# intcomp/camouflaged-vlm

Hardware: AMD Instinct MI355X
Metric: images/sec at 1024x1024 (SAM-ViT-H + CLIP ViT-L/14), full cascade (higher is better)
Workload: dtype f16 hi.hi MFMA + block-scaled e4m3 MFMA for the two correction products (3 mantissa bits) in the ViT-H qkv / lin1 / lin2 and CLIP MLP GEMMs; 3x f16 split MFMA in the other GEMMs; f32 accumulate; ViT-H attention: q.k^T = ONE f16 product (Q and K as single f16 values), P.v = 2x f16 (P a single f16, V

## Files before the change

camouflaged-vlm_amd/csrc/attention_win2.hip:

```cpp
#include <stdlib.h>
#include <type_traits>
#include "common.h"
#include "../../include/cvlm.h"

namespace {

constexpr float LOG2E = 1.4426950408889634f;
typedef float f32x2 __attribute__((ext_vector_type(2)));

template <int OFF>
__device__ __forceinline__ half4 lds_read_tr16(unsigned lds_addr) {
    half4 r;
    asm volatile("ds_read_b64_tr_b16 %0, %1 offset:%2" : "=v"(r) : "v"(lds_addr), "n"(OFF));
    return r;
}
__device__ __forceinline__ void lds_wait() {
    asm volatile("s_waitcnt lgkmcnt(0)" ::: "memory");
    __builtin_amdgcn_sched_barrier(0);
}
template <int N> __device__ __forceinline__ void wait_vm() { asm volatile("s_waitcnt vmcnt(%0)" ::"n"(N) : "memory"); }
__device__ __forceinline__ void step_barrier() {
    asm volatile("s_waitcnt lgkmcnt(0)" ::: "memory");
    __builtin_amdgcn_s_barrier();
    asm volatile("" ::: "memory");
}

struct OneHotImage2 { half_t v[224 * 32]; };
constexpr OneHotImage2 make_onehot_image2() {
    OneHotImage2 im{};
    for (int s = 0; s < 224; ++s)
        for (int c = 0; c < 32; ++c) {
            const int kh = s / 14, kw = s % 14;
            const bool one = s < 196 && (c == kh || c == 16 + kw);
            const int chunk = (c >> 3) ^ ((s >> 2) & 3);
            im.v[s * 32 + chunk * 8 + (c & 7)] = one ? (half_t)1.0f : (half_t)0.0f;
        }
    return im;
}
__device__ const OneHotImage2 g_onehot2 = make_onehot_image2();

#ifdef CVLM_PROBES
__device__ unsigned long long* g_win2_trace = nullptr;
#define WIN2_STAMP(x) do { if (trace) { __builtin_amdgcn_sched_barrier(0); x = wall_clock64(); __builtin_amdgcn_sched_barrier(0); } } while (0)
#else
#define WIN2_STAMP(x) do { } while (0)
#endif

template <bool PLO, bool QLO, bool KLO>
__global__ __launch_bounds__(512, 1) void attn_win14p_kernel(const cvlm_attn_args g, const int nwx, const int npairs) {
    constexpr int HD = 80, KS = 5, NDB = 5, CPR = 10, KP = 80, VP = 80, L = 14, S_SEQ = 196;
    constexpr int KT = 32, NKT = 7, NCW = 7;
    constexpr int PLANE_B = 5120, SLOT_B = 2 * PLANE_B, IPP = 5;
    constexpr int OFF_K = 0, OFF_V = 3 * SLOT_B, OFF_T = 6 * SLOT_B;
    constexpr int RT_B = 27 * HD * 2, RS_PIECES = (4 * RT_B + 1023) / 1024, RS_B = RS_PIECES * 1024;
    constexpr int OFF_OH = OFF_T + RS_B, OH_B = 224 * 32 * 2;
    constexpr int OFF_TOK = OFF_OH + OH_B, TOK_B = 2 * 224 * 8;
    constexpr int TP = 17, OFF_TAUG = OFF_TOK + 2 * TOK_B;

    extern __shared__ __attribute__((aligned(16))) unsigned char smem[];
    const int tid = threadIdx.x, lane = tid & 63;
    const int wave = __builtin_amdgcn_readfirstlane(tid >> 6);
    const int qc = lane & 31, half = lane >> 5;
    const int D = g.heads * HD;
    const half_t* qkv_hi = (const half_t*)g.qkv_hi;
    const half_t* qkv_lo = (const half_t*)g.qkv_lo;
    const half_t* pad_hi = (const half_t*)g.pad_hi;
    const half_t* pad_lo = (const half_t*)g.pad_lo;
    const int64_t qkv_plane = qkv_lo - qkv_hi, pad_plane = pad_lo - pad_hi;
    const int nwin = nwx * nwx;
    const int SI = g.grid * g.grid;
    const QkvStrides QS = qkv_strides(g.qkv_layout, SI, g.B, g.heads, HD);
    const int my_items = blockIdx.x < npairs ? (npairs - 1 - (int)blockIdx.x) / (int)gridDim.x + 1 : 0;
    const int T = my_items * NKT;
    auto pair_of = [&](int k) -> int { return (int)blockIdx.x + k * (int)gridDim.x; };
    auto token_of = [&](int pair, int slot) -> int {
        const int seq = pair / g.heads;
        const int w = seq % nwin;
        const int wy = w / nwx, wx = w - wy * nwx;
        const int iy = slot / L, ix = slot - iy * L;
        const int y = wy * L + iy, x = wx * L + ix;
        if (y >= g.grid || x >= g.grid) return -1;
        return y * g.grid + x;
    };

    if (wave == NCW) {
        long long* tokoff = (long long*)(smem + OFF_TOK);
        auto fill_tokoff = [&](int k) {
            const int pair = pair_of(k);
            const int head = pair % g.heads, b = (pair / g.heads) / nwin;
            long long* tk = tokoff + (k & 1) * (TOK_B / 8);
            const long long pad_delta = pad_hi - qkv_hi;
#pragma unroll
            for (int r = 0; r < 4; ++r) {
                const int sl = lane + 64 * r;
                if (sl < 224) {
                    const int tok = token_of(pair, sl < S_SEQ ? sl : S_SEQ - 1);
                    const long long ko = tok < 0 ? pad_delta + D + head * HD : (long long)qkv_offset(QS, b, tok, 1, head);
                    tk[sl] = ko | (tok < 0 ? 1 : 0);
                    tk[224 + sl] = (ko + (tok < 0 ? (long long)D : (long long)QS.sop)) | (tok < 0 ? 1 : 0);
                }
            }
            asm volatile("s_waitcnt lgkmcnt(0)" ::: "memory");
        };
        int row_s[IPP], ch_s[IPP];
#pragma unroll
        for (int sub = 0; sub < IPP; ++sub) {
            const int c = sub * 64 + lane;
            row_s[sub] = c / CPR;
            ch_s[sub] = c - row_s[sub] * CPR;
        }
        auto issue_tile = [&](int op, int gt) {
            const int k = gt / NKT, t = gt - k * NKT;
            const long long* tk = tokoff + (k & 1) * (TOK_B / 8) + op * 224 + t * KT;
            unsigned char* dst = smem + (op ? OFF_V : OFF_K) + (gt % 3) * SLOT_B;
            const half_t* src[IPP][2];
#pragma unroll
            for (int sub = 0; sub < IPP; ++sub) {
                const long long ko = tk[row_s[sub]];
                const long long disp = (ko & 1) ? pad_plane : qkv_plane;
                src[sub][0] = qkv_hi + ((ko & ~7ll) + ch_s[sub] * 8);
                src[sub][1] = src[sub][0] + disp;
            }
#pragma unroll
            for (int pl = 0; pl < 2; ++pl) {
                if (!KLO && pl == 1 && op == 0) continue;
#pragma unroll
                for (int sub = 0; sub < IPP; ++sub) glds16(src[sub][pl], dst + pl * PLANE_B + sub * 1024);
            }
        };
        {
            const unsigned char* t0 = (const unsigned char*)g.relh_hi;
            const unsigned char* t1 = (const unsigned char*)g.relh_lo;
            const unsigned char* t2 = (const unsigned char*)g.relw_hi;
            const unsigned char* t3 = (const unsigned char*)g.relw_lo;
#pragma unroll 1
            for (int i = 0; i < RS_PIECES; ++i) {
                int byte = i * 1024 + lane * 16;
                if (byte >= 4 * RT_B) byte = 0;
                const int tbl = byte / RT_B, off = byte - tbl * RT_B;
                const unsigned char* src = (tbl == 0 ? t0 : (tbl == 1 ? t1 : (tbl == 2 ? t2 : t3))) + off;
                glds16(src, smem + OFF_T + i * 1024);
            }
            const unsigned char* oh = (const unsigned char*)g_onehot2.v;
#pragma unroll 1
            for (int i = 0; i < OH_B / 1024; ++i) glds16(oh + i * 1024 + lane * 16, smem + OFF_OH + i * 1024);
        }
        if (T > 0) {
            fill_tokoff(0);
            issue_tile(0, 0);
            if (T > 1) issue_tile(0, 1);
            if (T > 2) issue_tile(0, 2);
            issue_tile(1, 0);
            if (T > 1) issue_tile(1, 1);
        }
        wait_vm<0>();
        step_barrier();
#pragma unroll 1
        for (int gt = 0; gt < T; ++gt) {
            step_barrier();
            const int kn = gt + 3, vn = gt + 2;
            if (kn < T && kn % NKT == 0) fill_tokoff(kn / NKT);
#if defined(CVLM_WIN2_PROBE) && CVLM_WIN2_PROBE == 2
            const bool ik = false, iv = false;
#else
            const bool ik = kn < T, iv = vn < T;
#endif
            if (ik) issue_tile(0, kn);
            if (iv) issue_tile(1, vn);
            constexpr int KB = (KLO ? 2 : 1) * IPP, VB = 2 * IPP;
            if (ik && iv) wait_vm<KB + VB>();
            else if (ik) wait_vm<KB>();
            else if (iv) wait_vm<VB>();
            else wait_vm<0>();
        }
        return;
    }

    float* Taug = (float*)(smem + OFF_TAUG);
    const half_t* OH = (const half_t*)(smem + OFF_OH);
    auto k_slot = [&](int gt) -> const unsigned char* { return smem + OFF_K + (gt % 3) * SLOT_B; };
    auto v_slot = [&](int gt) -> const unsigned char* { return smem + OFF_V + (gt % 3) * SLOT_B; };
    const int tg = lane >> 4, ti = lane & 15;
    const int v_lane_off = (16 * (tg & 1) + 4 * (tg >> 1) + (ti >> 2)) * VP + 4 * (ti & 3);
    typedef std::integral_constant<bool, false> no_c;
    typedef std::integral_constant<bool, true> yes_c;
    bool first = true;
    const int qslot = wave * 32 + qc;
    const bool qvalid = qslot < S_SEQ;
    const int qs = qvalid ? qslot : S_SEQ - 1;
    half8 qn_h[KS], qn_l[KS];
    auto load_q = [&](int pair) {
        const int head = pair % g.heads, b = (pair / g.heads) / nwin;
        const int qtok = token_of(pair, qs);
        const int64_t qo = qtok < 0 ? (int64_t)head * HD : qkv_offset(QS, b, qtok, 0, head);
        const half_t* bh = (qtok < 0 ? pad_hi : qkv_hi) + qo;
        const half_t* bl = bh + (qtok < 0 ? pad_plane : qkv_plane);
#pragma unroll
        for (int ks = 0; ks < KS; ++ks) {
            qn_h[ks] = *(const half8*)(bh + 16 * ks + 8 * half);
            qn_l[ks] = *(const half8*)(bl + 16 * ks + 8 * half);
        }
    };
    if (my_items > 0) load_q(pair_of(0));
#ifdef CVLM_PROBES
    unsigned long long* const trace = g_win2_trace;
    unsigned long long ta = 0, tb = 0, tc = 0, td = 0, acc_u = 0, acc_t = 0, acc_o = 0, acc_bar = 0, t_first = 0;
#endif

#pragma unroll 1
    for (int k = 0; k < my_items; ++k) {
        const int pair = pair_of(k);
        const int head = pair % g.heads, b = (pair / g.heads) / nwin;
        const int gt0 = k * NKT;
        half8 qh[KS + 2], ql[KS + 2];
#pragma unroll
        for (int ks = 0; ks < KS; ++ks) { qh[ks] = qn_h[ks]; ql[ks] = qn_l[ks]; }
        if (first) { step_barrier(); first = false; }
        WIN2_STAMP(ta);
        {
            const int qhh = qs / L, qww = qs - qhh * L;
            float* Tq = Taug + (wave * 32 + qc) * TP;
            if (half == 0) { Tq[14] = 0.f; Tq[15] = 0.f; }
            const int rr = qc < 27 ? qc : 26;
            floatx16 u[2];
#pragma unroll
            for (int tb = 0; tb < 2; ++tb) {
                const unsigned char* rt = smem + OFF_T + (2 * tb) * RT_B + rr * (HD * 2) + 16 * half;
#pragma unroll
                for (int r = 0; r < 16; ++r) u[tb][r] = 0.f;
#pragma unroll
                for (int ks = 0; ks < KS; ++ks) {
                    const half8 rh = *(const half8*)(rt + 32 * ks);
                    const half8 rl = *(const half8*)(rt + RT_B + 32 * ks);
                    u[tb] = __builtin_amdgcn_mfma_f32_32x32x16_f16(rh, qh[ks], u[tb], 0, 0, 0);
                    u[tb] = __builtin_amdgcn_mfma_f32_32x32x16_f16(rl, qh[ks], u[tb], 0, 0, 0);
                    u[tb] = __builtin_amdgcn_mfma_f32_32x32x16_f16(rh, ql[ks], u[tb], 0, 0, 0);
                }
            }
            if (g.scale != 1.0f) {
#pragma unroll
                for (int ks = 0; ks < KS; ++ks)
#pragma unroll
                    for (int j = 0; j < 8; ++j) {
                        half_t hh, ll;
                        split_h2(((float)qh[ks][j] + (float)ql[ks][j]) * g.scale, hh, ll);
                        qh[ks][j] = hh;
                        ql[ks][j] = ll;
                    }
            }
#pragma unroll
            for (int tb = 0; tb < 2; ++tb) {
                int cq = tb ? qww : qhh;
                asm volatile("" : "+v"(cq), "+v"(u[tb][0]));
#pragma unroll
                for (int r = 0; r < 16; ++r) {
                    const int j = (r & 3) + 8 * (r >> 2) + 4 * half;
                    const int kidx = cq + L - 1 - j;
                    const bool ok = j < 27 && kidx >= 0 && kidx < L;
                    Tq[ok ? kidx : 16] = u[tb][r];
                }
                __builtin_amdgcn_wave_barrier();
                {
                    typedef unsigned u32x4_s __attribute__((ext_vector_type(4)));
                    u32x4_s h4, l4;
#pragma unroll
                    for (int j = 0; j < 4; ++j) {
                        unsigned a, b;
                        split_h2_pk(Tq[8 * half + 2 * j], Tq[8 * half + 2 * j + 1], a, b);
                        h4[j] = a; l4[j] = b;
                    }
                    qh[KS + tb] = __builtin_bit_cast(half8, h4);
                    ql[KS + tb] = __builtin_bit_cast(half8, l4);
                }
                __builtin_amdgcn_wave_barrier();
            }
        }

        WIN2_STAMP(tb);
        float m_run = -INFINITY, l_run = 0.f;
        floatx4 o[NDB][2];
#pragma unroll
        for (int n = 0; n < NDB; ++n)
#pragma unroll
            for (int qb = 0; qb < 2; ++qb) o[n][qb] = floatx4{0.f, 0.f, 0.f, 0.f};
        floatx4 osum[2] = {floatx4{0.f, 0.f, 0.f, 0.f}, floatx4{0.f, 0.f, 0.f, 0.f}};

        auto scores = [&](int t, auto last_c) -> floatx16 {
            floatx16 s;
#pragma unroll
            for (int r = 0; r < 16; ++r) s[r] = 0.f;
            const half_t* kr = (const half_t*)k_slot(gt0 + t) + qc * KP + 8 * half;
#pragma unroll
            for (int ks = 0; ks < KS; ++ks) {
                const half8 kh = *(const half8*)(kr + 16 * ks);
                s = __builtin_amdgcn_mfma_f32_32x32x16_f16(kh, qh[ks], s, 0, 0, 0);
                if constexpr (KLO) {
                    const half8 kl = *(const half8*)(kr + PLANE_B / 2 + 16 * ks);
                    s = __builtin_amdgcn_mfma_f32_32x32x16_f16(kl, qh[ks], s, 0, 0, 0);
                }
                if constexpr (QLO) s = __builtin_amdgcn_mfma_f32_32x32x16_f16(kh, ql[ks], s, 0, 0, 0);
            }
            const int row = t * KT + qc;
            const half_t* ohr = OH + row * 32;
#pragma unroll
            for (int a = 0; a < 2; ++a) {
                const half8 oh8 = *(const half8*)(ohr + 8 * ((half + 2 * a) ^ ((row >> 2) & 3)));
                s = __builtin_amdgcn_mfma_f32_32x32x16_f16(oh8, qh[KS + a], s, 0, 0, 0);
                s = __builtin_amdgcn_mfma_f32_32x32x16_f16(oh8, ql[KS + a], s, 0, 0, 0);
            }
            if (decltype(last_c)::value) {
                const int b0 = t * KT + 4 * half;
#pragma unroll
                for (int r = 0; r < 16; ++r)
                    if (b0 + (r & 3) + 8 * (r >> 2) >= S_SEQ) s[r] = -INFINITY;
            }
            return s;
        };
        floatx16 s_cur = scores(0, no_c{});

        auto tile = [&](int t, auto has_next_c, auto next_last_c) {
            constexpr bool HAS_NEXT = decltype(has_next_c)::value;
#ifdef CVLM_PROBES
            unsigned long long te = 0, tf = 0;
            WIN2_STAMP(te);
#endif
            step_barrier();
#ifdef CVLM_PROBES
            WIN2_STAMP(tf);
            if (trace) acc_bar += tf - te;
#endif
#if defined(CVLM_WIN2_PROBE) && CVLM_WIN2_PROBE == 1
            return;
#endif
            floatx16 s_next;
            if (HAS_NEXT) s_next = scores(t + 1, next_last_c);
            const unsigned vaddr = (unsigned)(size_t)(LDS_AS const unsigned char*)v_slot(gt0 + t) + 2u * (unsigned)v_lane_off;
            auto read_v = [&](auto db_c, half4 (&v0)[2], half4 (&v1)[2]) {
                constexpr int DB = decltype(db_c)::value;
                v0[0] = lds_read_tr16<2 * (16 * DB)>(vaddr);                 v1[0] = lds_read_tr16<2 * (16 * DB + 8 * VP)>(vaddr);
                v0[1] = lds_read_tr16<PLANE_B + 2 * (16 * DB)>(vaddr);       v1[1] = lds_read_tr16<PLANE_B + 2 * (16 * DB + 8 * VP)>(vaddr);
            };
            half4 va0[3][2], va1[3][2], vb0[2][2], vb1[2][2];
            read_v(std::integral_constant<int, 0>{}, va0[0], va1[0]);
            read_v(std::integral_constant<int, 1>{}, va0[1], va1[1]);
            read_v(std::integral_constant<int, 2>{}, va0[2], va1[2]);
            const floatx16 s = s_cur;
            float mx = fmaxf(s[0], s[1]);
#pragma unroll
            for (int r = 2; r < 16; r += 2) mx = fmaxf(fmaxf(mx, s[r]), s[r + 1]);
            mx = half_swap_max(mx);
            constexpr float TAU = 5.0f;
            if (__builtin_amdgcn_ballot_w64(mx > m_run + TAU) != 0) {
                const float m_new = fmaxf(m_run, mx);
                const float alpha = __builtin_amdgcn_exp2f((m_run - m_new) * LOG2E);
                l_run *= alpha;
                const auto ax = __builtin_amdgcn_permlane16_swap(__builtin_bit_cast(unsigned, alpha), __builtin_bit_cast(unsigned, alpha), false, false);
                const float a0 = __builtin_bit_cast(float, (unsigned)ax[0]), a1 = __builtin_bit_cast(float, (unsigned)ax[1]);
#pragma unroll
                for (int n = 0; n < NDB; ++n) { o[n][0] *= a0; o[n][1] *= a1; }
                osum[0] *= a0; osum[1] *= a1;
                m_run = m_new;
            }
            const f32x2 c2 = f32x2{-m_run * LOG2E, -m_run * LOG2E}, l2 = f32x2{LOG2E, LOG2E};
            f32x2 z[8], acc = f32x2{0.f, 0.f};
#pragma unroll
            for (int i = 0; i < 8; ++i) {
                const f32x2 a = f32x2{s[2 * i], s[2 * i + 1]} * l2 + c2;
                z[i] = f32x2{__builtin_amdgcn_exp2f(a.x), __builtin_amdgcn_exp2f(a.y)};
                acc += z[i];
            }
            l_run += acc.x + acc.y;
            typedef unsigned u32x4 __attribute__((ext_vector_type(4)));
            u32x4 xh[2], xl[2];
#pragma unroll
            for (int p2 = 0; p2 < 4; ++p2) {
                const f32x2 e0 = z[p2], e1 = z[4 + p2];
                unsigned h0, h1;
                if constexpr (PLO) {
                    h0 = __builtin_bit_cast(unsigned, __builtin_amdgcn_cvt_pkrtz(e0.x, e0.y));
                    h1 = __builtin_bit_cast(unsigned, __builtin_amdgcn_cvt_pkrtz(e1.x, e1.y));
                    const half2v f0 = __builtin_bit_cast(half2v, h0), f1 = __builtin_bit_cast(half2v, h1);
                    const unsigned l0 = __builtin_bit_cast(unsigned, __builtin_amdgcn_cvt_pkrtz(e0.x - (float)f0[0], e0.y - (float)f0[1]));
                    const unsigned l1 = __builtin_bit_cast(unsigned, __builtin_amdgcn_cvt_pkrtz(e1.x - (float)f1[0], e1.y - (float)f1[1]));
                    const auto rl = __builtin_amdgcn_permlane16_swap(l0, l1, false, false);
                    xl[0][p2] = (unsigned)rl[0]; xl[1][p2] = (unsigned)rl[1];
                } else {
                    h0 = __builtin_bit_cast(unsigned, __builtin_convertvector(e0, half2v));
                    h1 = __builtin_bit_cast(unsigned, __builtin_convertvector(e1, half2v));
                }
                const auto rh = __builtin_amdgcn_permlane16_swap(h0, h1, false, false);
                xh[0][p2] = (unsigned)rh[0]; xh[1][p2] = (unsigned)rh[1];
            }
            auto pv = [&](int db, half4 (&v0)[2], half4 (&v1)[2]) {
                const half8 vh = half8{v0[0][0], v0[0][1], v0[0][2], v0[0][3], v1[0][0], v1[0][1], v1[0][2], v1[0][3]};
                const half8 vl = half8{v0[1][0], v0[1][1], v0[1][2], v0[1][3], v1[1][0], v1[1][1], v1[1][2], v1[1][3]};
#pragma unroll
                for (int qb = 0; qb < 2; ++qb) {
                    const half8 bh = __builtin_bit_cast(half8, xh[qb]), bl = __builtin_bit_cast(half8, xl[qb]);
                    if (!PLO && db == 0) {
                        const half_t one = (half_t)1.0f;
                        osum[qb] = __builtin_amdgcn_mfma_f32_16x16x32_f16(half8{one, one, one, one, one, one, one, one}, bh, osum[qb], 0, 0, 0);
                    }
                    o[db][qb] = __builtin_amdgcn_mfma_f32_16x16x32_f16(vh, bh, o[db][qb], 0, 0, 0);
                    o[db][qb] = __builtin_amdgcn_mfma_f32_16x16x32_f16(vl, bh, o[db][qb], 0, 0, 0);
                    if constexpr (PLO) o[db][qb] = __builtin_amdgcn_mfma_f32_16x16x32_f16(vh, bl, o[db][qb], 0, 0, 0);
                }
            };
            lds_wait();
            read_v(std::integral_constant<int, 3>{}, vb0[0], vb1[0]);
            read_v(std::integral_constant<int, 4>{}, vb0[1], vb1[1]);
            pv(0, va0[0], va1[0]);
            pv(1, va0[1], va1[1]);
            pv(2, va0[2], va1[2]);
            lds_wait();
            pv(3, vb0[0], vb1[0]);
            pv(4, vb0[1], vb1[1]);
            if (HAS_NEXT) s_cur = s_next;
        };
#pragma unroll 1
        for (int t = 0; t < NKT - 2; ++t) tile(t, yes_c{}, no_c{});
        tile(NKT - 2, yes_c{}, yes_c{});
        if (k + 1 < my_items) load_q(pair_of(k + 1));
        tile(NKT - 1, no_c{}, no_c{});
        WIN2_STAMP(tc);

        float invq[2];
        if constexpr (PLO) {
            const float l_tot = half_swap_sum(l_run);
            const float inv = 1.0f / l_tot;
            const auto ix = __builtin_amdgcn_permlane16_swap(__builtin_bit_cast(unsigned, inv), __builtin_bit_cast(unsigned, inv), false, false);
            invq[0] = __builtin_bit_cast(float, (unsigned)ix[0]); invq[1] = __builtin_bit_cast(float, (unsigned)ix[1]);
        } else {
            invq[0] = 1.0f / osum[0][0]; invq[1] = 1.0f / osum[1][0];
        }
        const int g4 = lane >> 4;
#pragma unroll
        for (int qb = 0; qb < 2; ++qb) {
            const int qs2 = wave * 32 + 16 * qb + (lane & 15);
            const int tok2 = token_of(pair, qs2 < S_SEQ ? qs2 : S_SEQ - 1);
            const bool ok2 = qs2 < S_SEQ && tok2 >= 0;
            const int64_t orow = ((int64_t)b * SI + (ok2 ? tok2 : 0)) * D + head * HD;
            half_t* oh = (half_t*)g.out_hi + orow;
            half_t* ol = (half_t*)g.out_lo + orow;
            unsigned ph2[NDB][2][2];
#pragma unroll
            for (int n = 0; n < NDB; ++n) {
                split_h2_pk(o[n][qb][0] * invq[qb], o[n][qb][1] * invq[qb], ph2[n][0][0], ph2[n][1][0]);
                split_h2_pk(o[n][qb][2] * invq[qb], o[n][qb][3] * invq[qb], ph2[n][0][1], ph2[n][1][1]);
            }
#pragma unroll
            for (int pl = 0; pl < 2; ++pl) {
                half_t* dst = pl ? ol : oh;
#pragma unroll
                for (int pr = 0; pr < 2; ++pr) {
                    const auto r0 = __builtin_amdgcn_permlane16_swap(ph2[2 * pr][pl][0], ph2[2 * pr + 1][pl][0], false, false);
                    const auto r1 = __builtin_amdgcn_permlane16_swap(ph2[2 * pr][pl][1], ph2[2 * pr + 1][pl][1], false, false);
                    typedef unsigned u32x4 __attribute__((ext_vector_type(4)));
                    const u32x4 v = u32x4{(unsigned)r0[0], (unsigned)r1[0], (unsigned)r0[1], (unsigned)r1[1]};
                    const int d = (g4 & 1) ? 16 * (2 * pr + 1) + 4 * (g4 - 1) : 16 * (2 * pr) + 4 * g4;
                    if (ok2) *(u32x4*)(dst + d) = v;
                }
                typedef unsigned u32x2 __attribute__((ext_vector_type(2)));
                if (ok2) *(u32x2*)(dst + 64 + 4 * g4) = u32x2{ph2[4][pl][0], ph2[4][pl][1]};
            }
        }
#ifdef CVLM_PROBES
        WIN2_STAMP(td);
        if (trace) { acc_u += tb - ta; acc_t += tc - tb; acc_o += td - tc; if (k == 0) t_first = ta; }
#endif
    }
#ifdef CVLM_PROBES
    if (trace && lane == 0) {
        unsigned long long* o = trace + ((size_t)blockIdx.x * 8 + wave) * 8;
        o[0] = acc_u; o[1] = acc_t; o[2] = acc_o; o[3] = (unsigned long long)my_items; o[4] = t_first; o[5] = td; o[6] = acc_bar;
        o[7] = __builtin_amdgcn_s_getreg((31 << 11) | 4);
    }
#endif
    if (first) step_barrier();
}

}

#ifdef CVLM_PROBES
extern "C" int cvlm_debug_set_attn_win2_trace(void* buf) { return (int)hipMemcpyToSymbol(HIP_SYMBOL(g_win2_trace), &buf, sizeof(buf)); }
#endif

template <bool PLO, bool QLO, bool KLO>
static int launch_win14(const cvlm_attn_args& g, hipStream_t s) {
    constexpr int smem = 6 * 10240 + 17 * 1024 + 224 * 32 * 2 + 2 * (2 * 224 * 8) + 224 * 17 * 4;
    const int nwx = (g.grid + 13) / 14;
    const int npairs = g.heads * g.B * nwx * nwx;
    static bool attr[16] = {};
    if (cvlm_first_on_device(attr))
        (void)hipFuncSetAttribute((const void*)attn_win14p_kernel<PLO, QLO, KLO>, hipFuncAttributeMaxDynamicSharedMemorySize, smem);
    static int cus_[16] = {};
    int dev = 0;
    (void)hipGetDevice(&dev);
    int& cus = cus_[dev & 15];
    if (cus == 0 && hipDeviceGetAttribute(&cus, hipDeviceAttributeMultiprocessorCount, dev) != hipSuccess) cus = 256;
    const int wgs = npairs < cus ? npairs : cus;
    hipLaunchKernelGGL((attn_win14p_kernel<PLO, QLO, KLO>), dim3(wgs), dim3(512), smem, s, g, nwx, npairs);
    CVLM_CHECK_LAUNCH();
    return 0;
}

int cvlm_attention_window14_pc(const cvlm_attn_args& g, hipStream_t s) {
    if (g.split_qk == 3 && g.split_pv == 3) return launch_win14<true, true, true>(g, s);
    if (g.split_qk == 2 && g.split_pv == 2) return launch_win14<false, false, true>(g, s);
    if (g.split_qk == 1 && g.split_pv == 2) return launch_win14<false, false, false>(g, s);
    return CVLM_E_UNSUPPORTED;
}
```

camouflaged-vlm_amd/hip.py:

```python
from __future__ import annotations

import ctypes as C
import functools
import os
from typing import Optional, Tuple

import torch

_PKG = os.path.dirname(os.path.abspath(__file__))
LIB_PATH = os.path.join(_PKG, "lib", "libcvlm_hip.so")

ACT_NONE, ACT_GELU, ACT_QUICKGELU, ACT_RELU, ACT_ABS_POST = 0, 1, 2, 3, 4

_SIGNATURES = {
    "cvlm_abi_version": "i:", "cvlm_target_arch": "z:",
    "cvlm_gemm": "i:Gs", "cvlm_gemm_workspace_bytes": "l:", "cvlm_debug_gemm_plan": "i:GiiI",
    "cvlm_layernorm": "i:plpipppfipppiis",
    "cvlm_add_rows": "i:ppifpppiis",
    "cvlm_ln_stats_merge": "i:pliifpps",
    "cvlm_row_stats_split": "i:pfpppliiils",
    "cvlm_row_stats_split_mx": "i:pfplplplpliiils",
    "cvlm_split_f32": "i:pppls",
    "cvlm_patchify": "i:pipiiiiippis",
    "cvlm_im2col3x3": "i:piiiipps",
    "cvlm_reinterpret_transpose": "i:piiifpps",
    "cvlm_attention": "i:As", "cvlm_attention_workspace_bytes": "l:A",
    "cvlm_small_attention": "i:plplplpliiiiis",
    "cvlm_small_attention_h2": "i:plplplplppliiiiis",
    "cvlm_dense_pe": "i:piips",
    "cvlm_mask_head": "i:pppiiips",
    "cvlm_mask_head_edge": "i:pppiiipps",
    "cvlm_mask_head_multi": "i:pppiiiipps",
    "cvlm_bilinear": "i:piiipiiis",
    "cvlm_clip_assemble": "i:ppppiiiips",
    "cvlm_overwrite_rows": "i:piiiiips",
    "cvlm_gather_rows": "i:piiipips",
    "cvlm_gather_rows_h2": "i:ppfiiipips",
    "cvlm_clip_head": "i:ppfiiipppps",
    "cvlm_topk_select": "i:piiipippps",
    "cvlm_text_assemble": "i:ppippipiiiips",
    "cvlm_clip_head_wide_workspace_bytes": "l:ii",
    "cvlm_clip_head_wide": "i:ppfiiipppppls",
    "cvlm_topk_select_wide": "i:piiipippps",
    "cvlm_expand_blocks": "i:piilpppppps",
    "cvlm_normalize_add": "i:ppiips",
    "cvlm_resample_u8": "i:piiiippiiips",
    "cvlm_u8_to_tensor": "i:piiiiiiiippps",
    "cvlm_mask_to_u8": "i:piiiiips",
    "cvlm_mask_joint_hist": "i:ppiiipps",
    "cvlm_mask_pack": "i:pilippps",
    "cvlm_mask_overlap": "i:piilps",
    "cvlm_mask_components_workspace_bytes": "l:iii",
    "cvlm_mask_components": "i:piiiiiiplpppppps",
    "cvlm_debug_mask_components_host": "i:piiiiiipppppp",
    "cvlm_mask_holes_workspace_bytes": "l:iii",
    "cvlm_mask_holes": "i:piiiiiiplppppps",
    "cvlm_debug_mask_holes_host": "i:piiiiiippppp",
    "cvlm_mask_wfm": "i:ppiiipppps",
    "cvlm_prob_quantise": "i:piiippps",
    "cvlm_prob_moments": "i:ppiiipppps",
    "cvlm_prob_wfm": "i:ppiiipppps",
    "cvlm_topk_accumulate": "i:ppiipps",
}
EXPORTS = list(_SIGNATURES)
ABI_VERSION = 12


class GemmArgs(C.Structure):
    _fields_ = [
        ("a_hi", C.c_void_p), ("a_lo", C.c_void_p), ("lda", C.c_int64), ("stride_a", C.c_int64),
        ("w_hi", C.c_void_p), ("w_lo", C.c_void_p), ("ldw", C.c_int64), ("stride_w", C.c_int64),
        ("bias", C.c_void_p),
        ("residual", C.c_void_p), ("ldr", C.c_int64), ("stride_r", C.c_int64),
        ("out_f32", C.c_void_p), ("ldo", C.c_int64), ("stride_o", C.c_int64),
        ("out_hi", C.c_void_p), ("out_lo", C.c_void_p), ("ldoh", C.c_int64), ("stride_oh", C.c_int64),
        ("M", C.c_int32), ("N", C.c_int32), ("K", C.c_int32), ("batch", C.c_int32),
        ("alpha", C.c_float), ("act", C.c_int32), ("split", C.c_int32),
        ("ps_h", C.c_int32), ("ps_w", C.c_int32), ("ps_c2", C.c_int32),
        ("hm_S", C.c_int32), ("hm_H", C.c_int32), ("hm_hd", C.c_int32),
        ("out_scale", C.c_float), ("workspace", C.c_void_p), ("workspace_bytes", C.c_int64),
        ("ln_stats", C.c_void_p), ("ln_colsum", C.c_void_p), ("ln_eps", C.c_float), ("ln_D", C.c_int32),
        ("res_hi", C.c_void_p), ("res_lo", C.c_void_p), ("ldrh", C.c_int64), ("res_scale", C.c_float),
        ("row_stats", C.c_void_p),
        ("conv_h", C.c_int32), ("conv_w", C.c_int32), ("conv_c", C.c_int32),
        ("w_il", C.c_void_p), ("ldw_il", C.c_int64),
        ("a_il", C.c_int32), ("out_il", C.c_int32), ("res_il", C.c_int32),
        ("a_mx", C.c_int32), ("out_mx", C.c_int32), ("res_mx", C.c_int32),
        ("a_mxs", C.c_void_p), ("lda_s", C.c_int64),
        ("w_mx", C.c_void_p), ("ldw_mx", C.c_int64), ("w_mxs", C.c_void_p), ("ldw_s", C.c_int64),
        ("out_mxs", C.c_void_p), ("ldo_s", C.c_int64), ("ldol", C.c_int64), ("ldrl", C.c_int64),
        ("hm_nolo", C.c_int32),
    ]


class GemmLaunchInfo(C.Structure):
    _fields_ = [(n, C.c_int32) for n in ("n0", "N", "nbx", "nby", "grid_x", "grid_y", "block", "lds_bytes", "group_m", "tail_rem",
                                         "tail_split", "total_blocks", "sk_parts", "uses_workspace")] + [("kernel", C.c_char * 128)]


class GemmPlanInfo(C.Structure):
    _fields_ = [("launches", C.c_int32), ("launch", GemmLaunchInfo * 2)]


class AttnArgs(C.Structure):
    _fields_ = [
        ("qkv_hi", C.c_void_p), ("qkv_lo", C.c_void_p), ("pad_hi", C.c_void_p), ("pad_lo", C.c_void_p),
        ("relh_hi", C.c_void_p), ("relh_lo", C.c_void_p), ("relw_hi", C.c_void_p), ("relw_lo", C.c_void_p),
        ("out_hi", C.c_void_p), ("out_lo", C.c_void_p),
        ("B", C.c_int32), ("S", C.c_int32), ("heads", C.c_int32), ("hd", C.c_int32),
        ("mode", C.c_int32), ("grid", C.c_int32), ("window", C.c_int32), ("causal", C.c_int32),
        ("split_qk", C.c_int32), ("split_pv", C.c_int32), ("scale", C.c_float), ("qkv_layout", C.c_int32),
        ("workspace", C.c_void_p), ("workspace_bytes", C.c_int64), ("q_rows", C.c_int32),
    ]


_CTYPES = {"i": C.c_int32, "l": C.c_int64, "f": C.c_float, "p": C.c_void_p, "s": C.c_void_p, "z": C.c_char_p,
           "G": C.POINTER(GemmArgs), "A": C.POINTER(AttnArgs), "I": C.POINTER(GemmPlanInfo)}
ABI = {name: (_CTYPES[sig[0]], [_CTYPES[c] for c in sig[2:]]) for name, sig in _SIGNATURES.items()}
_STREAMED = frozenset(name for name, sig in _SIGNATURES.items() if sig.endswith("s"))

_lib: Optional[C.CDLL] = None


def load() -> C.CDLL:
    global _lib
    if _lib is not None:
        return _lib
    path = os.environ.get("CVLM_PROBE_LIB") or LIB_PATH
    if not os.path.exists(path):
        raise RuntimeError(
            f"{path} is missing: the HIP kernels are the only compute path of this package. "
            "Build them with `python -c 'import __graft_entry__ as g; g.build()'` (hipcc --offload-arch=gfx950).")
    lib = C.CDLL(path)
    for name, (restype, argtypes) in ABI.items():
        fn = getattr(lib, name)
        fn.restype, fn.argtypes = restype, argtypes
    if lib.cvlm_abi_version() != ABI_VERSION:
        raise RuntimeError(f"{path}: ABI {lib.cvlm_abi_version()}, this binding needs {ABI_VERSION}: rebuild the library")
    _lib = lib
    return lib


def _check(rc: int, what: str) -> None:
    if rc != 0:
        raise RuntimeError(f"{what} failed with code {rc}")


def _p(t: Optional[torch.Tensor]) -> Optional[int]:
    return None if t is None else t.data_ptr()


def _planes(x: Optional["H2"]) -> Tuple[Optional[int], Optional[int]]:
    return (None, None) if x is None else (x.hi.data_ptr(), x.lo.data_ptr())


def _stream() -> Optional[int]:
    return torch.cuda.current_stream().cuda_stream or None


def _call(name: str, *args) -> None:
    fn = getattr(load(), name)
    _check(fn(*args, _stream()) if name in _STREAMED else fn(*args), name)


def _on_current_device(t: torch.Tensor) -> None:
    if t.device.type != "cuda" or t.device.index != torch.cuda.current_device():
        raise RuntimeError(f"tensor on {t.device}, current device is cuda:{torch.cuda.current_device()}: call "
                           "torch.cuda.set_device() first (launches use the current device's stream)")


def gemm_workspace_bytes() -> int:
    return load().cvlm_gemm_workspace_bytes()


def new_gemm_workspace(device) -> torch.Tensor:
    return torch.zeros(gemm_workspace_bytes(), dtype=torch.uint8, device=device)


def gemm_workspace_errors(ws: torch.Tensor) -> int:
# ... 607 lines not shown
```

include/cvlm.h:

```cpp
#ifndef CVLM_H
#define CVLM_H
#include <stdint.h>
#ifdef __cplusplus
extern "C" {
#endif

#define CVLM_ABI_VERSION 12
#define CVLM_E_BADARG (-1)
#define CVLM_E_UNSUPPORTED (-2)
#define CVLM_E_WORKSPACE (-3)

enum { CVLM_ACT_NONE = 0, CVLM_ACT_GELU = 1, CVLM_ACT_QUICKGELU = 2, CVLM_ACT_RELU = 3, CVLM_ACT_ABS_POST = 4 };

int cvlm_abi_version(void);
const char* cvlm_target_arch(void);

typedef struct cvlm_gemm_args {
    const void* a_hi; const void* a_lo; int64_t lda; int64_t stride_a;
    const void* w_hi; const void* w_lo; int64_t ldw; int64_t stride_w;
    const float* bias;
    const float* residual; int64_t ldr; int64_t stride_r;
    float* out_f32; int64_t ldo; int64_t stride_o;
    void* out_hi; void* out_lo; int64_t ldoh; int64_t stride_oh;
    int32_t M, N, K, batch;
    float alpha;
    int32_t act;
    int32_t split;
    int32_t ps_h, ps_w, ps_c2;
    int32_t hm_S, hm_H, hm_hd;
    float out_scale;
    void* workspace;
    int64_t workspace_bytes;
    const float* ln_stats; const float* ln_colsum; float ln_eps; int32_t ln_D;
    const void* res_hi; const void* res_lo; int64_t ldrh; float res_scale;
    float* row_stats;
    int32_t conv_h, conv_w, conv_c;
    const void* w_il; int64_t ldw_il;
    int32_t a_il, out_il, res_il;
    int32_t a_mx, out_mx, res_mx;
    const void* a_mxs; int64_t lda_s;
    const void* w_mx; int64_t ldw_mx; const void* w_mxs; int64_t ldw_s;
    void* out_mxs; int64_t ldo_s; int64_t ldol; int64_t ldrl;
    int32_t hm_nolo;
} cvlm_gemm_args;
int cvlm_gemm(const cvlm_gemm_args* args, void* stream);
int64_t cvlm_gemm_workspace_bytes(void);
typedef struct cvlm_gemm_plan_info {
    int32_t launches;
    struct {
        int32_t n0, N;
        int32_t nbx, nby, grid_x, grid_y, block, lds_bytes;
        int32_t group_m, tail_rem, tail_split, total_blocks, sk_parts, uses_workspace;
        char kernel[128];
    } launch[2];
} cvlm_gemm_plan_info;
int cvlm_debug_gemm_plan(const cvlm_gemm_args* args, int have_ws, int cus, cvlm_gemm_plan_info* out);

int cvlm_layernorm(const float* x, int64_t ldx, const float* add, int32_t add_rows, float* sum_out,
                   const float* gamma, const float* beta, float eps, int32_t act,
                   float* out_f32, void* out_hi, void* out_lo, int32_t M, int32_t D, void* stream);

int cvlm_add_rows(const float* a, const float* b, int32_t b_rows, float scale, float* out_f32,
                  void* out_hi, void* out_lo, int32_t M, int32_t D, void* stream);

#define CVLM_LN_FOLD_MAX_RATIO 128
#define CVLM_WS_WORD_LN_REFUSED 513
int cvlm_ln_stats_merge(const float* pieces, int64_t piece_rows, int32_t M, int32_t D, float eps, float* merged, void* gemm_workspace,
                        void* stream);

int cvlm_row_stats_split(const float* x, float scale, void* out_hi, void* out_lo, float* stats, int64_t stats_rows, int32_t M,
                         int32_t D, int32_t copies, int64_t dst_row_stride, void* stream);
int cvlm_row_stats_split_mx(const float* x, float scale, void* out_img, int64_t ld_img, void* out_scales, int64_t ld_s, void* out_lo,
                            int64_t ld_lo, float* stats, int64_t stats_rows, int32_t M, int32_t D, int32_t copies, int64_t dst_row_stride,
                            void* stream);

int cvlm_split_f32(const float* x, void* out_hi, void* out_lo, int64_t n, void* stream);

int cvlm_patchify(const float* src0, int32_t C0, const float* src1, int32_t C1, int32_t B, int32_t H,
                  int32_t W, int32_t p, void* out_hi, void* out_lo, int32_t ldk, void* stream);

int cvlm_im2col3x3(const float* x, int32_t B, int32_t H, int32_t W, int32_t C, void* out_hi, void* out_lo,
                   void* stream);

int cvlm_reinterpret_transpose(const float* x, int32_t B, int32_t T, int32_t D, float scale, void* out_hi, void* out_lo,
                               void* stream);

typedef struct cvlm_attn_args {
    const void* qkv_hi; const void* qkv_lo;
    const void* pad_hi; const void* pad_lo;
    const void* relh_hi; const void* relh_lo;
    const void* relw_hi; const void* relw_lo;
    void* out_hi; void* out_lo;
    int32_t B, S, heads, hd;
    int32_t mode, grid, window, causal;
    int32_t split_qk, split_pv;
    float scale;
    int32_t qkv_layout;
    void* workspace;
    int64_t workspace_bytes;
    int32_t q_rows;
} cvlm_attn_args;
int cvlm_attention(const cvlm_attn_args* args, void* stream);
int64_t cvlm_attention_workspace_bytes(const cvlm_attn_args* args);

int cvlm_small_attention(const float* q, int64_t ldq, const float* k, int64_t ldk, const float* v, int64_t ldv,
                         float* out, int64_t ldo, int32_t B, int32_t nq, int32_t nk, int32_t heads, int32_t hd,
                         void* stream);
int cvlm_small_attention_h2(const float* q, int64_t ldq, const float* k, int64_t ldk, const float* v, int64_t ldv, float* out, int64_t ldo,
                            void* out_hi, void* out_lo, int64_t ldoh, int32_t B, int32_t nq, int32_t nk, int32_t heads, int32_t hd,
                            void* stream);

int cvlm_dense_pe(const float* gauss, int32_t size, int32_t C, float* out, void* stream);

int cvlm_mask_head(const float* up, const float* edge_emb, const float* hyper, int32_t B, int32_t HW, int32_t C,
                   float* low, void* stream);

int cvlm_mask_head_edge(const float* up, const float* edge_emb, const float* hyper, int32_t P, int32_t HW, int32_t C,
                        float* low, float* edge_prob, void* stream);

int cvlm_mask_head_multi(const float* up, const float* edge_emb, const float* hyper, int32_t P, int32_t HW, int32_t C,
                         int32_t n_masks, float* low, float* edge_prob, void* stream);

int cvlm_bilinear(const float* in, int32_t N, int32_t hin, int32_t win, float* out, int32_t hout, int32_t wout,
                  int32_t sigmoid_in, void* stream);

int cvlm_clip_assemble(const float* patches, const float* cls, const float* pos, const float* ctx,
                       int32_t B, int32_t P, int32_t W, int32_t nctx, float* out, void* stream);

int cvlm_overwrite_rows(float* x, int32_t B, int32_t L, int32_t W, int32_t first, int32_t n, const float* src,
                        void* stream);

int cvlm_gather_rows(const float* x, int32_t B, int32_t L, int32_t W, const int32_t* idx, int32_t fixed,
                     float* out, void* stream);
int cvlm_gather_rows_h2(const void* x_hi, const void* x_lo, float scale, int32_t B, int32_t L, int32_t W, const int32_t* idx,
                        int32_t fixed, float* out, void* stream);

int cvlm_clip_head(const float* img, const float* txt, float logit_scale_exp, int32_t B, int32_t C, int32_t D,
                   float* img_n, float* logits, int64_t* pred, float* txt_sel, void* stream);

int cvlm_topk_select(const float* logits, int32_t B, int32_t C, int32_t K, const float* txt, int32_t D, const int64_t* idx_in,
                     int64_t* idx_out, float* sel, void* stream);

int cvlm_text_assemble(const int32_t* ids, const float* table, int32_t V, const float* emb, const float* ctx, int32_t n_ctx,
                       const float* pos, int32_t n, int32_t ctx_len, int32_t L, int32_t W, float* out, void* stream);

int64_t cvlm_clip_head_wide_workspace_bytes(int32_t P, int32_t C);
int cvlm_clip_head_wide(const float* img, const float* txt, float logit_scale_exp, int32_t P, int32_t C, int32_t D, float* img_n,
                        float* logits, int64_t* pred, float* txt_sel, void* workspace, int64_t workspace_bytes, void* stream);

int cvlm_topk_select_wide(const float* logits, int32_t B, int32_t C, int32_t K, const float* txt, int32_t D, const int64_t* idx_in,
                          int64_t* idx_out, float* sel, void* stream);

int cvlm_expand_blocks(const int32_t* image_of, int32_t P, int32_t B, int64_t block_elems, const float* src_f32, float* dst_f32,
                       const void* src_hi, const void* src_lo, void* dst_hi, void* dst_lo, void* stream);

int cvlm_normalize_add(const float* x, const float* add, int32_t R, int32_t D, float* out, void* stream);

int cvlm_resample_u8(const uint8_t* src, int32_t N, int32_t H, int32_t W, int32_t C, const int32_t* bounds,
                     const int32_t* kk, int32_t ksize, int32_t n_out, int32_t axis, uint8_t* dst, void* stream);

int cvlm_u8_to_tensor(const uint8_t* src, int32_t N, int32_t H, int32_t W, int32_t C, int32_t top, int32_t left,
                      int32_t ch, int32_t cw, const float* mean, const float* stdv, float* dst, void* stream);

int cvlm_mask_to_u8(const float* logits, int32_t N, int32_t Hs, int32_t Ws, int32_t h, int32_t w, uint8_t* dst, void* stream);

int cvlm_mask_joint_hist(const uint8_t* pre, const uint8_t* gt, int32_t N, int32_t h, int32_t w, uint64_t* stats, uint32_t* hist,
                         void* stream);

int cvlm_mask_pack(const float* logits, int32_t P, int64_t HW, int32_t W, uint8_t* bits, int32_t* area, int32_t* box, void* stream);

int cvlm_mask_overlap(const uint32_t* bits, int32_t n, int32_t K, int64_t words, int32_t* inter, void* stream);

int64_t cvlm_mask_components_workspace_bytes(int32_t P, int32_t H, int32_t W);
int cvlm_mask_components(const uint32_t* bits, int32_t P, int32_t H, int32_t W, int32_t connectivity, int32_t M, int32_t min_area,
                         void* workspace, int64_t workspace_bytes, int32_t* n_comp, int32_t* comps, int32_t* n_kept, uint32_t* kept_bits,
                         int32_t* kept_area, int32_t* kept_box, void* stream);
int cvlm_debug_mask_components_host(const uint32_t* bits, int32_t P, int32_t H, int32_t W, int32_t connectivity, int32_t M,
                                    int32_t min_area, int32_t* n_comp, int32_t* comps, int32_t* n_kept, uint32_t* kept_bits,
                                    int32_t* kept_area, int32_t* kept_box);

int64_t cvlm_mask_holes_workspace_bytes(int32_t P, int32_t H, int32_t W);
int cvlm_mask_holes(const uint32_t* bits, int32_t P, int32_t H, int32_t W, int32_t connectivity, int32_t M, int32_t fill_below,
                    void* workspace, int64_t workspace_bytes, int32_t* n_holes, int32_t* holes, int32_t* n_filled,
                    uint32_t* filled_bits, int32_t* filled_area, void* stream);
int cvlm_debug_mask_holes_host(const uint32_t* bits, int32_t P, int32_t H, int32_t W, int32_t connectivity, int32_t M,
                               int32_t fill_below, int32_t* n_holes, int32_t* holes, int32_t* n_filled, uint32_t* filled_bits,
                               int32_t* filled_area);

int cvlm_mask_wfm(const uint8_t* pre, const uint8_t* gt, int32_t N, int32_t h, int32_t w, const uint32_t* hist,
                  const double* gauss49, void* workspace, double* out3, void* stream);

int cvlm_prob_quantise(const float* prob, int32_t N, int32_t h, int32_t w, float* minmax, uint8_t* q, void* workspace, void* stream);
int cvlm_prob_moments(const float* prob, const uint8_t* gt, int32_t N, int32_t h, int32_t w, const float* minmax, const uint64_t* stats,
                      void* workspace, double* out, void* stream);
int cvlm_prob_wfm(const float* prob, const uint8_t* gt, int32_t N, int32_t h, int32_t w, const float* minmax, const double* gauss49,
                  void* workspace, double* out3, void* stream);

int cvlm_topk_accumulate(const float* scores, const int32_t* labels, int32_t B, int32_t C, int32_t* pred, uint32_t* counters,
                         void* stream);

#ifdef __cplusplus
}
#endif
#endif
```

Measured before the change: 64.92.

## Pack real query tokens in padded windows and trim last key tile softmax

Queries in edge windows are now packed so only real (unpadded) tokens occupy wave slots, and waves with no real queries skip compute and only join the tile barriers. The final key tile's softmax is limited to its 4 valid rows: the masking loop is dropped and exp/convert work is halved, with one half-wave forced to zero. This cuts wasted MFMA and exp work on padded windows. It adds per-pair geometry arithmetic and relies on the last tile holding at most 4 valid keys per lane group.

Result: no change. 65.05 (median of 6 runs) (+0.2%).

```diff
diff --git a/camouflaged-vlm_amd/csrc/attention_win2.hip b/camouflaged-vlm_amd/csrc/attention_win2.hip
--- a/camouflaged-vlm_amd/csrc/attention_win2.hip
+++ b/camouflaged-vlm_amd/csrc/attention_win2.hip
@@ -2,6 +2,13 @@
 #include <type_traits>
 #include "common.h"
 #include "../../include/cvlm.h"
+
+#ifndef CVLM_WIN2_PACKQ
+#define CVLM_WIN2_PACKQ 1
+#endif
+#ifndef CVLM_WIN2_LAST4
+#define CVLM_WIN2_LAST4 1
+#endif
 
 namespace {
 
@@ -185,13 +192,39 @@
     typedef std::integral_constant<bool, false> no_c;
     typedef std::integral_constant<bool, true> yes_c;
     bool first = true;
-    const int qslot = wave * 32 + qc;
-    const bool qvalid = qslot < S_SEQ;
-    const int qs = qvalid ? qslot : S_SEQ - 1;
+    constexpr bool PACKQ = CVLM_WIN2_PACKQ != 0;
+    constexpr bool LAST4 = CVLM_WIN2_LAST4 != 0 && !PLO;
+    struct QGeo { int y0, x0, cols, mul, nreal; };
+    auto geo_of = [&](int pair) -> QGeo {
+        const int w = (pair / g.heads) % nwin;
+        const int wy = w / nwx, wx = w - wy * nwx;
+        QGeo q{wy * L, wx * L, L, 65536 / L + 1, S_SEQ};
+        if (PACKQ) {
+            const int rows = min(L, g.grid - q.y0);
+            q.cols = min(L, g.grid - q.x0);
+            q.mul = 65536 / q.cols + 1;
+            q.nreal = rows * q.cols;
+        }
+        return q;
+    };
+    auto qpos = [&](const QGeo& q, int i, int& iy, int& ix) {
+        i = min(i, q.nreal - 1);
+        iy = PACKQ ? (i * q.mul) >> 16 : i / L;
+        ix = i - iy * q.cols;
+    };
+    auto qtoken = [&](const QGeo& q, int i) -> int {
+        int iy, ix;
+        qpos(q, i, iy, ix);
+        const int y = q.y0 + iy, x = q.x0 + ix;
+        if (!PACKQ && (y >= g.grid || x >= g.grid)) return -1;
+        return y * g.grid + x;
+    };
     half8 qn_h[KS], qn_l[KS];
     auto load_q = [&](int pair) {
+        const QGeo q = geo_of(pair);
+        if (wave * 32 >= q.nreal) return;
         const int head = pair % g.heads, b = (pair / g.heads) / nwin;
-        const int qtok = token_of(pair, qs);
+        const int qtok = qtoken(q, wave * 32 + qc);
         const int64_t qo = qtok < 0 ? (int64_t)head * HD : qkv_offset(QS, b, qtok, 0, head);
         const half_t* bh = (qtok < 0 ? pad_hi : qkv_hi) + qo;
         const half_t* bl = bh + (qtok < 0 ? pad_plane : qkv_plane);
@@ -212,13 +245,21 @@
         const int pair = pair_of(k);
         const int head = pair % g.heads, b = (pair / g.heads) / nwin;
         const int gt0 = k * NKT;
+        const QGeo gq = geo_of(pair);
+        if (first) { step_barrier(); first = false; }
+        if (wave * 32 >= gq.nreal) {
+            if (k + 1 < my_items) load_q(pair_of(k + 1));
+#pragma unroll 1
+            for (int t = 0; t < NKT; ++t) step_barrier();
+            continue;
+        }
         half8 qh[KS + 2], ql[KS + 2];
 #pragma unroll
         for (int ks = 0; ks < KS; ++ks) { qh[ks] = qn_h[ks]; ql[ks] = qn_l[ks]; }
-        if (first) { step_barrier(); first = false; }
         WIN2_STAMP(ta);
         {
-            const int qhh = qs / L, qww = qs - qhh * L;
+            int qhh, qww;
+            qpos(gq, wave * 32 + qc, qhh, qww);
             float* Tq = Taug + (wave * 32 + qc) * TP;
             if (half == 0) { Tq[14] = 0.f; Tq[15] = 0.f; }
             const int rr = qc < 27 ? qc : 26;
@@ -308,7 +349,7 @@
                 s = __builtin_amdgcn_mfma_f32_32x32x16_f16(oh8, qh[KS + a], s, 0, 0, 0);
                 s = __builtin_amdgcn_mfma_f32_32x32x16_f16(oh8, ql[KS + a], s, 0, 0, 0);
             }
-            if (decltype(last_c)::value) {
+            if (!LAST4 && decltype(last_c)::value) {
                 const int b0 = t * KT + 4 * half;
 #pragma unroll
                 for (int r = 0; r < 16; ++r)
@@ -320,6 +361,8 @@
 
         auto tile = [&](int t, auto has_next_c, auto next_last_c) {
             constexpr bool HAS_NEXT = decltype(has_next_c)::value;
+            constexpr bool FOUR = LAST4 && !HAS_NEXT;
+            constexpr int NZ = FOUR ? 2 : 8, NP = FOUR ? 2 : 4;
 #ifdef CVLM_PROBES
             unsigned long long te = 0, tf = 0;
             WIN2_STAMP(te);
@@ -347,7 +390,8 @@
             const floatx16 s = s_cur;
             float mx = fmaxf(s[0], s[1]);
 #pragma unroll
-            for (int r = 2; r < 16; r += 2) mx = fmaxf(fmaxf(mx, s[r]), s[r + 1]);
+            for (int r = 2; r < 2 * NZ; r += 2) mx = fmaxf(fmaxf(mx, s[r]), s[r + 1]);
+            if (FOUR && half) mx = -INFINITY;
             mx = half_swap_max(mx);
             constexpr float TAU = 5.0f;
             if (__builtin_amdgcn_ballot_w64(mx > m_run + TAU) != 0) {
@@ -361,22 +405,24 @@
                 osum[0] *= a0; osum[1] *= a1;
                 m_run = m_new;
             }
-            const f32x2 c2 = f32x2{-m_run * LOG2E, -m_run * LOG2E}, l2 = f32x2{LOG2E, LOG2E};
-            f32x2 z[8], acc = f32x2{0.f, 0.f};
-#pragma unroll
-            for (int i = 0; i < 8; ++i) {
+            const float c1 = (FOUR && half) ? -INFINITY : -m_run * LOG2E;
+            const f32x2 c2 = f32x2{c1, c1}, l2 = f32x2{LOG2E, LOG2E};
+            f32x2 z[NZ], acc = f32x2{0.f, 0.f};
+#pragma unroll
+            for (int i = 0; i < NZ; ++i) {
                 const f32x2 a = f32x2{s[2 * i], s[2 * i + 1]} * l2 + c2;
                 z[i] = f32x2{__builtin_amdgcn_exp2f(a.x), __builtin_amdgcn_exp2f(a.y)};
                 acc += z[i];
             }
             l_run += acc.x + acc.y;
             typedef unsigned u32x4 __attribute__((ext_vector_type(4)));
-            u32x4 xh[2], xl[2];
-#pragma unroll
-            for (int p2 = 0; p2 < 4; ++p2) {
-                const f32x2 e0 = z[p2], e1 = z[4 + p2];
-                unsigned h0, h1;
+            u32x4 xh[2] = {u32x4{0, 0, 0, 0}, u32x4{0, 0, 0, 0}}, xl[2] = {u32x4{0, 0, 0, 0}, u32x4{0, 0, 0, 0}};
+#pragma unroll
+            for (int p2 = 0; p2 < NP; ++p2) {
+                const f32x2 e0 = z[p2];
+                unsigned h0, h1 = 0;
                 if constexpr (PLO) {
+                    const f32x2 e1 = z[4 + p2];
                     h0 = __builtin_bit_cast(unsigned, __builtin_amdgcn_cvt_pkrtz(e0.x, e0.y));
                     h1 = __builtin_bit_cast(unsigned, __builtin_amdgcn_cvt_pkrtz(e1.x, e1.y));
                     const half2v f0 = __builtin_bit_cast(half2v, h0), f1 = __builtin_bit_cast(half2v, h1);
@@ -386,7 +432,7 @@
                     xl[0][p2] = (unsigned)rl[0]; xl[1][p2] = (unsigned)rl[1];
                 } else {
                     h0 = __builtin_bit_cast(unsigned, __builtin_convertvector(e0, half2v));
-                    h1 = __builtin_bit_cast(unsigned, __builtin_convertvector(e1, half2v));
+                    if constexpr (!FOUR) h1 = __builtin_bit_cast(unsigned, __builtin_convertvector(z[NZ / 2 + p2], half2v));
                 }
                 const auto rh = __builtin_amdgcn_permlane16_swap(h0, h1, false, false);
                 xh[0][p2] = (unsigned)rh[0]; xh[1][p2] = (unsigned)rh[1];
@@ -437,8 +483,8 @@
 #pragma unroll
         for (int qb = 0; qb < 2; ++qb) {
             const int qs2 = wave * 32 + 16 * qb + (lane & 15);
-            const int tok2 = token_of(pair, qs2 < S_SEQ ? qs2 : S_SEQ - 1);
-            const bool ok2 = qs2 < S_SEQ && tok2 >= 0;
+            const int tok2 = qtoken(gq, qs2);
+            const bool ok2 = qs2 < gq.nreal && tok2 >= 0;
             const int64_t orow = ((int64_t)b * SI + (ok2 ? tok2 : 0)) * D + head * HD;
             half_t* oh = (half_t*)g.out_hi + orow;
             half_t* ol = (half_t*)g.out_lo + orow;
```

## Pack real query slots first in edge windows and skip all-padding waves

Applied to the files above, without the earlier changes.

For edge windows that extend past the grid, query slots are reordered so real tokens come first and padding slots last. A compute wave whose 32 query rows are all padding then skips the QK/PV work and only joins the barriers to stay in step with the loader wave. It also adds a debug export of the slot mapping and probe counters for edge windows. This removes wasted MFMA work on padded queries in SAM's 64x64 grid with 14x14 windows, at the cost of extra index math and a possible load imbalance between waves.

Result: no change. 65.30 before, 65.36 after, median of 4 (+0.1%).

```diff
diff --git a/camouflaged-vlm_amd/csrc/attention_win2.hip b/camouflaged-vlm_amd/csrc/attention_win2.hip
--- a/camouflaged-vlm_amd/csrc/attention_win2.hip
+++ b/camouflaged-vlm_amd/csrc/attention_win2.hip
@@ -1,6 +1,7 @@
 #include <stdlib.h>
 #include <type_traits>
 #include "common.h"
+#include "attn_win_slots.h"
 #include "../../include/cvlm.h"
 
 namespace {
@@ -82,6 +83,20 @@
         if (y >= g.grid || x >= g.grid) return -1;
         return y * g.grid + x;
     };
+    auto win_of = [&](int pair) -> int {
+        const int w = (pair / g.heads) % nwin;
+        const int wy = w / nwx, wx = w - wy * nwx;
+        return __builtin_amdgcn_readfirstlane(wy | wx << 8 | cvlm_attn_win::real_extent(g.grid, nwx, wy) << 16 |
+                                              cvlm_attn_win::real_extent(g.grid, nwx, wx) << 24);
+    };
+    auto qtoken_of = [&](int wq, int slot) -> int {
+        const cvlm_attn_win::Pos p = cvlm_attn_win::query_pos(slot, (wq >> 16) & 255, wq >> 24);
+        const int y = (wq & 255) * L + p.iy, x = ((wq >> 8) & 255) * L + p.ix;
+        if (y >= g.grid || x >= g.grid) return -1;
+        return y * g.grid + x;
+    };
+    auto wave_active = [&](int wq) -> bool { return wave * 32 < ((wq >> 16) & 255) * (wq >> 24); };
+    auto next_active = [&](int k) -> bool { return k + 1 < my_items && wave_active(win_of(pair_of(k + 1))); };
 
     if (wave == NCW) {
         long long* tokoff = (long long*)(smem + OFF_TOK);
@@ -191,7 +206,7 @@
     half8 qn_h[KS], qn_l[KS];
     auto load_q = [&](int pair) {
         const int head = pair % g.heads, b = (pair / g.heads) / nwin;
-        const int qtok = token_of(pair, qs);
+        const int qtok = qtoken_of(win_of(pair), qs);
         const int64_t qo = qtok < 0 ? (int64_t)head * HD : qkv_offset(QS, b, qtok, 0, head);
         const half_t* bh = (qtok < 0 ? pad_hi : qkv_hi) + qo;
         const half_t* bl = bh + (qtok < 0 ? pad_plane : qkv_plane);
@@ -201,10 +216,10 @@
             qn_l[ks] = *(const half8*)(bl + 16 * ks + 8 * half);
         }
     };
-    if (my_items > 0) load_q(pair_of(0));
+    if (my_items > 0 && wave_active(win_of(pair_of(0)))) load_q(pair_of(0));
 #ifdef CVLM_PROBES
     unsigned long long* const trace = g_win2_trace;
-    unsigned long long ta = 0, tb = 0, tc = 0, td = 0, acc_u = 0, acc_t = 0, acc_o = 0, acc_bar = 0, t_first = 0;
+    unsigned long long ta = 0, tb = 0, tc = 0, td = 0, acc_u = 0, acc_t = 0, acc_o = 0, acc_bar = 0, t_first = 0, acc_edge = 0, n_edge = 0;
 #endif
 
 #pragma unroll 1
@@ -212,13 +227,22 @@
         const int pair = pair_of(k);
         const int head = pair % g.heads, b = (pair / g.heads) / nwin;
         const int gt0 = k * NKT;
+        const int wq = win_of(pair);
+        if (first) { step_barrier(); first = false; }
+        if (!wave_active(wq)) {
+#pragma unroll 1
+            for (int t = 0; t < NKT - 1; ++t) step_barrier();
+            if (next_active(k)) load_q(pair_of(k + 1));
+            step_barrier();
+            continue;
+        }
         half8 qh[KS + 2], ql[KS + 2];
 #pragma unroll
         for (int ks = 0; ks < KS; ++ks) { qh[ks] = qn_h[ks]; ql[ks] = qn_l[ks]; }
-        if (first) { step_barrier(); first = false; }
         WIN2_STAMP(ta);
         {
-            const int qhh = qs / L, qww = qs - qhh * L;
+            const cvlm_attn_win::Pos qp = cvlm_attn_win::query_pos(qs, (wq >> 16) & 255, wq >> 24);
+            const int qhh = qp.iy, qww = qp.ix;
             float* Tq = Taug + (wave * 32 + qc) * TP;
             if (half == 0) { Tq[14] = 0.f; Tq[15] = 0.f; }
             const int rr = qc < 27 ? qc : 26;
@@ -420,7 +444,7 @@
 #pragma unroll 1
         for (int t = 0; t < NKT - 2; ++t) tile(t, yes_c{}, no_c{});
         tile(NKT - 2, yes_c{}, yes_c{});
-        if (k + 1 < my_items) load_q(pair_of(k + 1));
+        if (next_active(k)) load_q(pair_of(k + 1));
         tile(NKT - 1, no_c{}, no_c{});
         WIN2_STAMP(tc);
 
@@ -437,7 +461,7 @@
 #pragma unroll
         for (int qb = 0; qb < 2; ++qb) {
             const int qs2 = wave * 32 + 16 * qb + (lane & 15);
-            const int tok2 = token_of(pair, qs2 < S_SEQ ? qs2 : S_SEQ - 1);
+            const int tok2 = qtoken_of(wq, qs2 < S_SEQ ? qs2 : S_SEQ - 1);
             const bool ok2 = qs2 < S_SEQ && tok2 >= 0;
             const int64_t orow = ((int64_t)b * SI + (ok2 ? tok2 : 0)) * D + head * HD;
             half_t* oh = (half_t*)g.out_hi + orow;
@@ -466,7 +490,11 @@
         }
 #ifdef CVLM_PROBES
         WIN2_STAMP(td);
-        if (trace) { acc_u += tb - ta; acc_t += tc - tb; acc_o += td - tc; if (k == 0) t_first = ta; }
+        if (trace) {
+            acc_u += tb - ta; acc_t += tc - tb; acc_o += td - tc;
+            if (k == 0) t_first = ta;
+            if (((wq >> 16) & 255) * (wq >> 24) < S_SEQ) { acc_edge += td - ta; ++n_edge; }
+        }
 #endif
     }
 #ifdef CVLM_PROBES
@@ -474,6 +502,7 @@
         unsigned long long* o = trace + ((size_t)blockIdx.x * 8 + wave) * 8;
         o[0] = acc_u; o[1] = acc_t; o[2] = acc_o; o[3] = (unsigned long long)my_items; o[4] = t_first; o[5] = td; o[6] = acc_bar;
         o[7] = __builtin_amdgcn_s_getreg((31 << 11) | 4);
+        if (wave == 0) { o[56] = acc_edge; o[59] = n_edge; }
     }
 #endif
     if (first) step_barrier();
@@ -484,6 +513,21 @@
 #ifdef CVLM_PROBES
 extern "C" int cvlm_debug_set_attn_win2_trace(void* buf) { return (int)hipMemcpyToSymbol(HIP_SYMBOL(g_win2_trace), &buf, sizeof(buf)); }
 #endif
+
+extern "C" int cvlm_debug_attn_win_query_slots(int32_t grid, int32_t window, int32_t wy, int32_t wx, int32_t* out) {
+    namespace W = cvlm_attn_win;
+    if (window != W::L || grid < 1 || !out) return CVLM_E_UNSUPPORTED;
+    const int nwx = (grid + W::L - 1) / W::L;
+    if (wy < 0 || wx < 0 || wy >= nwx || wx >= nwx) return CVLM_E_UNSUPPORTED;
+    const int rh = W::real_extent(grid, nwx, wy), rw = W::real_extent(grid, nwx, wx);
+    out[0] = rh * rw;
+    for (int s = 0; s < W::SLOTS; ++s) {
+        const W::Pos p = W::query_pos(s, rh, rw);
+        out[1 + 2 * s] = p.iy;
+        out[2 + 2 * s] = p.ix;
+    }
+    return 0;
+}
 
 template <bool PLO, bool QLO, bool KLO>
 static int launch_win14(const cvlm_attn_args& g, hipStream_t s) {
diff --git a/camouflaged-vlm_amd/csrc/attn_win_slots.h b/camouflaged-vlm_amd/csrc/attn_win_slots.h
--- /dev/null
+++ b/camouflaged-vlm_amd/csrc/attn_win_slots.h
@@ -0,0 +1,21 @@
+#pragma once
+
+namespace cvlm_attn_win {
+
+constexpr int L = 14, SLOTS = L * L;
+
+struct Pos { int iy, ix; };
+
+constexpr int real_extent(int grid, int nwx, int w) { return w + 1 < nwx ? L : grid - L * (nwx - 1); }
+
+constexpr Pos query_pos(int s, int rh, int rw) {
+    if (rw == L) { const int iy = s / L; return Pos{iy, s - iy * L}; }
+    const int nq = rh * rw;
+    if (s < nq) { const int iy = s / rw; return Pos{iy, s - iy * rw}; }
+    const int pw = L - rw, side = rh * pw, j = s - nq;
+    if (j < side) { const int iy = j / pw; return Pos{iy, rw + j - iy * pw}; }
+    const int iy = (j - side) / L;
+    return Pos{rh + iy, j - side - iy * L};
+}
+
+}
diff --git a/camouflaged-vlm_amd/hip.py b/camouflaged-vlm_amd/hip.py
--- a/camouflaged-vlm_amd/hip.py
+++ b/camouflaged-vlm_amd/hip.py
@@ -25,6 +25,7 @@
     "cvlm_im2col3x3": "i:piiiipps",
     "cvlm_reinterpret_transpose": "i:piiifpps",
     "cvlm_attention": "i:As", "cvlm_attention_workspace_bytes": "l:A",
+    "cvlm_debug_attn_win_query_slots": "i:iiiip",
     "cvlm_small_attention": "i:plplplpliiiiis",
     "cvlm_small_attention_h2": "i:plplplplppliiiiis",
     "cvlm_dense_pe": "i:piips",
diff --git a/include/cvlm.h b/include/cvlm.h
--- a/include/cvlm.h
+++ b/include/cvlm.h
@@ -101,6 +101,7 @@
     int32_t q_rows;
 } cvlm_attn_args;
 int cvlm_attention(const cvlm_attn_args* args, void* stream);
+int cvlm_debug_attn_win_query_slots(int32_t grid, int32_t window, int32_t wy, int32_t wx, int32_t* out);
 int64_t cvlm_attention_workspace_bytes(const cvlm_attn_args* args);
 
 int cvlm_small_attention(const float* q, int64_t ldq, const float* k, int64_t ldk, const float* v, int64_t ldv,
```
